# KyleVanMeter/MVOLPS

Hardware: AMD Instinct MI355X
Metric: simplex_pivots_per_s (higher is better)
Workload: dtype f64

## Files before the change

### mvolps_amd/csrc/kernels.hip

```cpp
#include <hip/hip_runtime.h>

#include <cmath>
#include <cstdlib>

#include "kernel_common.hpp"

namespace mvx {

template <int MODE>
__device__ __forceinline__ bool cand_better(const Cand &a, const Cand &b) {
  if (a.idx == 0) return false;
  if (b.idx == 0) return true;
  if (MODE == 0) {
    if (a.k1 > b.k1) return true;
    if (a.k1 < b.k1) return false;
    return a.idx < b.idx;
  } else {
    if (a.k1 < b.k1) return true;
    if (a.k1 > b.k1) return false;
    if (a.k2 > b.k2) return true;
    if (a.k2 < b.k2) return false;
    return a.idx < b.idx;
  }
}
// ... 2389 lines not shown
          if ((spc >> sx) & 1u) {                                                                                        \
            const double ips = s_ip[sx], pvs = s_piv[sx];                                                                \
            _Pragma("unroll") for (int u = 0; u < RPT; u++) a[u] = (ii[u] == lp8[k]) ? ips : xdiv(hc8[u][k], pvs);       \
          } else {                                                                                                       \
            _Pragma("unroll") for (int u = 0; u < RPT; u++) a[u] = (ii[u] == lp8[k]) ? -sq8[k] : fma(-hc8[u][k], sq8[k], a[u]); \
          }                                                                                                              \
        }                                                                                                                \
      }                                                                                                                  \
    }                                                                                                                    \
    s0 += N;                                                                                                             \
  }
      while (gu - s0 >= 8) { COL_BLOCK(8) }
      COL_BLOCK(4)
      COL_BLOCK(2)
      COL_BLOCK(1)
#undef COL_BLOCK
    }
    CH_STAMP(1);
    Cand rb{0.0, 0.0, 0, 0};
    double rp[4] = {a[0], be[0], lb[0], ub[0]}, ro[4];
#pragma unroll
    for (int u = 0; u < RPT; u++) {
      Cand x{0.0, 0.0, 0, 0};
      if (ii[u] <= m) {
        A.colq0[(size_t)g * A.cstride + ii[u]] = a[u];
        if (ratio_row(a[u], sdir, be[u], lb[u], ub[u], 0, A.tol_piv, ii[u], x) && cand_better<1>(x, rb)) {
          rb = x;
          rp[0] = a[u]; rp[1] = be[u]; rp[2] = lb[u]; rp[3] = ub[u];
        }
      }
      HC(g, u) = a[u];
    }
    CH_STAMP(2);
    const Cand pw = xchg<1, 4>(X, rb, rp, ro, s_slots, s_pay);
    if (X.dead) break;
    CH_STAMP(3);
    const int p = pw.idx, p_up = pw.aux;
    const double tstep = pw.k1, piv = ro[0], bp = ro[1], plb = ro[2], pub = ro[3];
    double val[CPT];
#pragma unroll
    for (int u = 0; u < CPT; u++) val[u] = T[(size_t)p * ld + ((jj[u] <= n) ? jj[u] : n)];
    double rcp_l = 0.0;
    if (lane < g) rcp_l = ld_sc1(A.colq0 + (size_t)lane * A.cstride + p);
    bool flip = false;
    double tf = 0.0;
    if (lbq > -INFINITY && ubq < INFINITY && fq != MVX_NF) {
      tf = ubq - lbq;
      if (p == 0 || tf <= tstep) flip = true;
    }
    if (!flip && p == 0) {
      if (lead && g == 0) {
        c->fstate = F_STOP;
        c->phase = PH_PRIMAL2;
      }
      break;
    }
    int kind, lf, stall_new;
    double delta = 0.0, bound = 0.0, s0 = 0.0, xq = 0.0, ip = 1.0;
    if (flip) {
      kind = ST_FLIP;
      lf = (sdir > 0) ? MVX_NU : MVX_NL;
      delta = (sdir > 0) ? tf : -tf;
      stall_new = 0;
#pragma unroll
      for (int u = 0; u < RPT; u++) be[u] = fma(a[u], delta, be[u]);
      z = fma(dq, delta, z);
#pragma unroll
      for (int u = 0; u < CPT; u++) {
        if (jj[u] == q) f[u] = lf;
        sqn[u] = 0.0;
      }
    } else {
      kind = ST_PIVOT;
      bound = p_up ? pub : plb;
      lf = dev_leave_flag(plb, pub, p_up);
      s0 = xdiv(bp - bound, piv);
      xq = dev_nb_value(fq, lbq, ubq);
      ip = xdiv(1.0, piv);
      stall_new = (tstep <= DEGEN_TOL) ? stall + 1 : 0;
#pragma unroll
      for (int u = 0; u < RPT; u++) {
        if (ii[u] == p) {
          be[u] = xq - s0;
          lb[u] = lbq;
          ub[u] = ubq;
        } else
          be[u] = fma(-a[u], s0, be[u]);
      }
      CH_STAMP(4);
      if (lane < g) {
        const double rcp = rcp_l;
        s_wv[wave][0][lane] = rcp;
        s_wv[wave][1][lane] = xdiv(rcp, s_piv[lane]);
      }
      const unsigned spr = (unsigned)__ballot(ispc && s_p[lane < KCH ? lane : 0] == p);
      {
        int s0 = 0;
#define ROW_BLOCK(N)                                                                                                     \
  if (gu - s0 >= N) {                                                                                                    \
    const unsigned bm = ((1u << N) - 1u) << s0;                                                                          \
    double hs8[CPT][N], cp8[N], cd8[N];                                                                                  \
    int lq8[N];                                                                                                          \
    _Pragma("unroll") for (int k = 0; k < N; k++) {                                                                      \
      cp8[k] = s_wv[wave][0][s0 + k];                                                                                    \
      cd8[k] = s_wv[wave][1][s0 + k];                                                                                    \
      lq8[k] = s_q[s0 + k];                                                                                              \
      _Pragma("unroll") for (int u = 0; u < CPT; u++) hs8[u][k] = HS(s0 + k, u);                                         \
    }                                                                                                                    \
    if ((pivm & bm) == bm && (spr & bm) == 0u) {                                                                         \
      _Pragma("unroll") for (int k = 0; k < N; k++) {                                                                    \
        _Pragma("unroll") for (int u = 0; u < CPT; u++) val[u] = (jj[u] == lq8[k]) ? cd8[k] : fma(-cp8[k], hs8[u][k], val[u]); \
      }                                                                                                                  \
    } else {                                                                                                             \
      _Pragma("unroll") for (int k = 0; k < N; k++) {                                                                    \
        const int sx = s0 + k;                                                                                           \
        if ((pivm >> sx) & 1u) {                                                                                         \
          if ((spr >> sx) & 1u) {                                                                                        \
            const double ips = s_ip[sx];                                                                                 \
            _Pragma("unroll") for (int u = 0; u < CPT; u++) val[u] = (jj[u] == lq8[k]) ? ips : -hs8[u][k];               \
          } else {                                                                                                       \
            _Pragma("unroll") for (int u = 0; u < CPT; u++) val[u] = (jj[u] == lq8[k]) ? cd8[k] : fma(-cp8[k], hs8[u][k], val[u]); \
          }                                                                                                              \
        }                                                                                                                \
      }                                                                                                                  \
    }                                                                                                                    \
    s0 += N;                                                                                                             \
  }
        while (gu - s0 >= 8) { ROW_BLOCK(8) }
        ROW_BLOCK(4)
        ROW_BLOCK(2)
        ROW_BLOCK(1)
#undef ROW_BLOCK
      }
      CH_STAMP(5);
#pragma unroll
      for (int u = 0; u < CPT; u++) {
        const int j = jj[u];
        const double sj = xdiv(val[u], piv);
        if (j == q) {
          d[u] = xdiv(dq, piv);
          const double cc = xdiv(wq, piv * piv);
          wgt[u] = cc > 1.0 ? cc : 1.0;
          lbj[u] = plb;
          ubj[u] = pub;
          f[u] = lf;
        } else {
          d[u] = fma(-dq, sj, d[u]);
          const double cc = sj * sj * wq;
          wgt[u] = cc > wgt[u] ? cc : wgt[u];
        }
        if (j <= n) A.srow0[(size_t)g * A.sstride + j] = sj;
        HS(g, u) = sj;
        sqn[u] = sj;
      }
      z = fma(-dq, s0, z);
      if (lead) A.srow0[(size_t)g * A.sstride] = s0;
    }
    s_kind[g] = kind;
    s_p[g] = flip ? 0 : p;
    s_q[g] = q;
    s_piv[g] = flip ? 1.0 : piv;
    s_ip[g] = ip;
    used += flip ? 0 : 1;
    if (lead) {
      c->ch_kind[g] = kind;
      c->ch_p[g] = flip ? 0 : p;
      c->ch_q[g] = q;
      c->ch_lf[g] = lf;
      c->ch_piv[g] = flip ? 1.0 : piv;
      c->ch_xq[g] = xq;
      c->ch_s0[g] = s0;
      c->ch_delta[g] = delta;
      c->ch_elb[g] = lbq;
      c->ch_eub[g] = ubq;
      c->ch_llb[g] = plb;
      c->ch_lub[g] = pub;
      c->ch_bound[g] = bound;
      c->ch_pup[g] = p_up;
      c->ch_stall[g] = stall_new;
      c->ch_cnt[g] = used;
      c->ch_ok[g] = epoch;
    }
    CH_STAMP(6);
    PRICE();
    CH_STAMP(7);
    stall = stall_new;
    g++;
    qc = xchg<0, 5>(X, pc, pp, po, s_slots, s_pay);
    if (dbg && lead) dbg[(size_t)(g - 1) * 16 + 8] = __builtin_amdgcn_s_memrealtime();
  }
#undef PRICE
#undef CH_STAMP
#undef HS
#undef HC
  if (X.dead) {
    if (lead) {
      c->pc_n = 0;
      c->cl_abort = 1;
    }
    return;
  }
  if (g == 0 && fresh) {
#pragma unroll
    for (int u = 0; u < CPT; u++) {
      if (jj[u] <= n) {
        A.pw[0][jj[u]] = 1.0;
        A.pw[1][jj[u]] = 1.0;
      }
    }
  }
  if (g > 0) {
    const int xf = g & 1;
#pragma unroll
    for (int u = 0; u < CPT; u++) {
      if (jj[u] <= n) {
        A.drowk[xf][jj[u]] = d[u];
        A.pwk[xf][jj[u]] = wgt[u];
      }
    }
    if (lead) {
      A.drowk[xf][0] = z;
      A.pwk[xf][0] = 1.0;
    }
  }
  if (lead) {
    c->pc_n = g;
    if (g > 0) {
      c->phase = PH_PRIMAL2;
      c->pc_itlim = end_itlim ? 1 : 0;
    }
  }
}

__device__ void chain_commit(const ChainArgs &A, Ctl *c, int nch) {
  __shared__ int s_cp[KCH], s_cq[KCH], s_ck[KCH], s_rf[KCH], s_cf[KCH], s_R[KCH], s_C[KCH];
  const int t = TIDX;
  const bool on = (t < nch);
  int kind = 0, p = 0, q = 0;
  if (on) {
    kind = c->ch_kind[t];
    p = c->ch_p[t];
    q = c->ch_q[t];
    s_ck[t] = kind;
    s_cp[t] = p;
    s_cq[t] = q;
    s_R[t] = (kind == ST_PIVOT) ? c->bvar[p] : 0;
    s_C[t] = (kind == ST_PIVOT) ? c->nvar[q] : 0;
  }
  __syncthreads();
  bool lastrow = true, lastcol = true, lastflag = true;
  if (on) {
    int rf = t, cf = t;
    for (int u = t - 1; u >= 0; u--) {
      if (s_ck[u] != ST_PIVOT) continue;
      if (s_cp[u] == p) rf = u;
      if (s_cq[u] == q) cf = u;
    }
    s_rf[t] = rf;
    s_cf[t] = cf;
    for (int u = t + 1; u < nch; u++) {
      if (s_cq[u] == q) lastflag = false;
      if (s_ck[u] != ST_PIVOT) continue;
      if (s_cp[u] == p) lastrow = false;
      if (s_cq[u] == q) lastcol = false;
    }
  }
  __syncthreads();
  if (t == 0) {
    for (int u = 0; u < nch; u++) {
      if (s_ck[u] != ST_PIVOT) continue;
      const int a = s_rf[u], b = s_cf[u];
      const int kv = s_R[a];
      s_R[a] = s_C[b];
      s_C[b] = kv;
    }
  }
  __syncthreads();
  if (on) {
    if (kind == ST_PIVOT) {
      if (lastrow) {
        c->bvar[p] = s_R[s_rf[t]];
        A.blb[p] = c->ch_elb[t];
        A.bub[p] = c->ch_eub[t];
      }
      if (lastcol) {
        c->nvar[q] = s_C[s_cf[t]];
        A.nlb[q] = c->ch_llb[t];
        A.nub[q] = c->ch_lub[t];
      }
    }
    if (lastflag) A.nflag[q] = c->ch_lf[t];
  }
  if (t == 0) {
    const int piv_n = c->ch_cnt[nch - 1];
    c->it_cnt += piv_n;
    c->n_flips += nch - piv_n;
    c->n_bulk++;
    if (c->budget > 0) c->budget -= piv_n;
    c->stall = c->ch_stall[nch - 1];
    c->pc_epoch++;
  }
}

typedef const double __attribute__((address_space(4))) *kconst_f64;
template <int TR, int NT>
__global__ __launch_bounds__(256) void k_fbc3(const ChainArgs A) {
  __shared__ double s_cq[KCH][TR];
  Ctl *const c = A.c;
  if (c->done != D_RUN || c->fstate != F_RUN) return;
  const int nch = c->pc_n;
  if (nch == 0) return;
  const int n = A.n;
  const size_t ld = (size_t)A.ld;
  const int j0 = 2 * ((int)blockIdx.x * 256 + TIDX);
  const int i0 = 1 + (int)blockIdx.y * TR;
  const int xf = nch & 1;
  const bool act = (j0 <= n);
  const int jc = act ? j0 : 0;
  double *base = A.T + (size_t)i0 * ld + jc;
  double2 v[TR];
#pragma unroll
  for (int r = 0; r < TR; r++) v[r] = ld2<NT>(reinterpret_cast<const double2 *>(base + (size_t)r * ld));
  unsigned flips = 0;
  for (int l = 0; l < nch; l++) flips |= (c->ch_kind[l] == ST_FLIP) ? (1u << l) : 0u;
  for (int e = TIDX; e < nch * TR; e += 256) {
    const int l = e / TR, r = e % TR;
    s_cq[l][r] = ((flips >> l) & 1u) ? 0.0 : A.colq0[(size_t)l * A.cstride + i0 + r];
  }
  __syncthreads();
  const double *sp = A.srow0 + jc;
  const double *zp = A.zeros + jc;
  for (int l0 = 0; l0 < nch; l0 += 4) {
    double2 s4[4];
#pragma unroll
    for (int k = 0; k < 4; k++) {
      const int lk = (l0 + k < nch) ? l0 + k : nch - 1;
      s4[k] = *reinterpret_cast<const double2 *>(((flips >> lk) & 1u) ? zp : sp + (size_t)lk * A.sstride);
    }
#pragma unroll
    for (int k = 0; k < 4; k++) {
      if (l0 + k < nch) {
#pragma unroll
        for (int r = 0; r < TR; r++) {
          const double ci = s_cq[l0 + k][r];
          asm("v_fma_f64 %0, -%1, %2, %0" : "+v"(v[r].x) : "v"(ci), "v"(s4[k].x));
          asm("v_fma_f64 %0, -%1, %2, %0" : "+v"(v[r].y) : "v"(ci), "v"(s4[k].y));
        }
      }
    }
  }
  if (act) {
    if (j0 == 0) {
#pragma unroll
      for (int r = 0; r < TR; r++) base[(size_t)r * ld + 1] = v[r].y;
    } else {
#pragma unroll
      for (int r = 0; r < TR; r++) st2<NT>(reinterpret_cast<double2 *>(base + (size_t)r * ld), v[r]);
    }
    if (blockIdx.y == 0) {
      *reinterpret_cast<double2 *>(A.T + j0) = *reinterpret_cast<const double2 *>(A.drowk[xf] + j0);
      const double2 w = *reinterpret_cast<const double2 *>(A.pwk[xf] + j0);
      *reinterpret_cast<double2 *>(A.pw[0] + j0) = w;
      *reinterpret_cast<double2 *>(A.pw[1] + j0) = w;
    }
  }
  if (blockIdx.x == 0 && blockIdx.y == 0) chain_commit(A, c, nch);
}

__global__ __launch_bounds__(256) void k_fpatch(const ChainArgs A, int kmax) {
  __shared__ int s_kind[KCH], s_p[KCH], s_q[KCH];
  __shared__ double s_piv[KCH], s_ip[KCH], s_xq[KCH], s_delta[KCH], s_u[KCH];
  Ctl *const c = A.c;
  if (c->done != D_RUN || c->fstate != F_RUN) return;
  const int nch = c->pc_n;
  if (nch == 0) return;
  const int m = A.m, n = A.n;
  const size_t ld = (size_t)A.ld;
  const int job = (int)blockIdx.y, x = (int)blockIdx.x * 256 + TIDX;
  const int jk = (job < kmax) ? 0 : (job < 2 * kmax) ? 1 : 2;
  const int l = (jk == 0) ? job : (jk == 1) ? job - kmax : -1;
  bool live = (jk == 2) || (l < nch && c->ch_kind[l < nch ? l : 0] == ST_PIVOT);
  const int span = (jk == 0) ? n : (jk == 1) ? m : A.mcap1 - 1;
  if ((int)blockIdx.x * 256 > span) live = false;
  if (live) {
    const int lp = (l >= 0) ? c->ch_p[l] : 0, lq = (l >= 0) ? c->ch_q[l] : 0;
    if (TIDX < KCH) {
      const int t = (TIDX < nch) ? TIDX : nch - 1;
      const int kind = c->ch_kind[t];
      const double piv = c->ch_piv[t];
      s_kind[TIDX] = kind;
      s_p[TIDX] = c->ch_p[t];
      s_q[TIDX] = c->ch_q[t];
      s_piv[TIDX] = piv;
      s_ip[TIDX] = (kind == ST_PIVOT) ? xdiv(1.0, piv) : 0.0;
      s_xq[TIDX] = c->ch_xq[t];
      s_delta[TIDX] = c->ch_delta[t];
      s_u[TIDX] = (jk == 0) ? A.colq0[(size_t)t * A.cstride + lp] : A.srow0[(size_t)t * A.sstride + (jk == 1 ? lq : 0)];
    }
    const int xc = (x >= 1 && x <= span) ? x : 1;
    double op[KCH];
#pragma unroll
    for (int t = 0; t < KCH; t++) {
      const int tc = (t < nch) ? t : nch - 1;
      op[t] = (jk == 0) ? A.srow0[(size_t)tc * A.sstride + xc] : A.colq0[(size_t)tc * A.cstride + xc];
    }
    double *dst = (jk == 0) ? A.T + (size_t)lp * ld + xc : A.T + (size_t)xc * ld + (jk == 1 ? lq : 0);
    double val = (jk == 2) ? *dst : 0.0;
    __syncthreads();
    const int i = (jk == 0) ? lp : xc, j = (jk == 0) ? xc : (jk == 1) ? lq : 0;
    const int l0 = (jk == 2) ? 0 : l;
#pragma unroll
    for (int t = 0; t < KCH; t++) {
      if (t >= l0 && t < nch) {
        const double ci = (jk == 0) ? s_u[t] : op[t], sj = (jk == 0) ? op[t] : s_u[t];
        if (s_kind[t] == ST_FLIP) {
          if (j == 0) val = fma(ci, s_delta[t], val);
        } else if (i == s_p[t]) {
          val = (j == s_q[t]) ? s_ip[t] : (j == 0) ? s_xq[t] - sj : -sj;
        } else if (j == s_q[t]) {
          val = xdiv(ci, s_piv[t]);
        } else {
          val = fma(-ci, sj, val);
        }
      }
    }
    if (x >= 1 && x <= span) {
      if (jk != 2 || x <= m) *dst = val;
      if (jk == 2) A.betab[x] = val;
    }
  }
}

__device__ __forceinline__ bool row_violation(double beta, double lb, double ub, double tol, double &viol, int &up) {
  viol = 0.0;
  up = 0;
  if (lb > -INFINITY && beta < lb - tol * (1.0 + fabs(lb))) viol = lb - beta;
  if (ub < INFINITY && beta > ub + tol * (1.0 + fabs(ub))) {
    viol = beta - ub;
    up = 1;
  }
  return viol > 0.0;
}

__device__ __forceinline__ bool dual_ratio_col(double a, double d, int f, int to_upper, double tp, int j, Cand &x) {
  if (f == MVX_NS) return false;
  const double aa = to_upper ? -a : a;
  double r;
  if (aa > tp && (f == MVX_NL || f == MVX_NF)) r = (f == MVX_NF) ? fabs(d) : (d < 0.0 ? -d : 0.0);
  else if (aa < -tp && (f == MVX_NU || f == MVX_NF)) r = (f == MVX_NF) ? fabs(d) : (d > 0.0 ? d : 0.0);
  else return false;
  const double mag = fabs(a);
  x = Cand{xdiv(r, mag), mag, j, 0};
  return true;
}

__global__ __launch_bounds__(DA_THREADS) void k_dboot(Ctl *c) {
  __shared__ Cand lds[17];
  const bool lead = (blockIdx.x == 0 && TIDX == 0);
  if (c->done != D_RUN || c->phase != PH_DUAL || c->stall >= c->stall_limit || c->perturbed) {
    if (lead) c->fstate = F_OFF;
    return;
  }
  const int a = c->curA & 1, m = c->m, n = c->n;
  const size_t ld = (size_t)c->ld;
  const double *T = c->T, *w = c->dwx[a];
  const double tol = c->tol_bnd;
  Cand rb{0.0, 0.0, 0, 0};
  for (int i = 1 + TIDX; i <= m; i += DA_THREADS) {
    double viol;
    int up;
    if (row_violation(T[(size_t)i * ld], c->blb[i], c->bub[i], tol, viol, up)) {
      Cand x{xdiv(viol * viol, w[i]), 0.0, i, up};
      if (cand_better<0>(x, rb)) rb = x;
    }
  }
  rb = block_best<0>(rb, lds);
  const int p2 = rb.idx, p2_up = rb.aux;
  const int j = (int)blockIdx.x * DA_THREADS + TIDX;
  Cand best{0.0, 0.0, 0, 0};
  if (p2 && j >= 1 && j <= n) {
    Cand x{0.0, 0.0, 0, 0};
    if (dual_ratio_col(T[(size_t)p2 * ld + j], c->sgn * T[j], c->nflag[j], p2_up, c->tol_piv, j, x)) best = x;
  }
  __syncthreads();
  best = block_best<1>(best, lds);
  if (TIDX == 0) c->pp[a][blockIdx.x] = best;
  if (lead) {
    c->p_nextx[a] = p2;
    c->p_up_nextx[a] = p2_up;
    c->fstate = F_RUN_DUAL;
    c->step = ST_NONE;
    c->curB = a ^ 1;
    c->npbd = (int)gridDim.x;
  }
}

__global__ __launch_bounds__(DA_THREADS) void k_da(Ctl *c) {
  __shared__ Cand lds[17];
  const int done = c->done, fstate = c->fstate, cur = c->curA, budget = c->budget;
  const int stall = c->stall, stall_limit = c->stall_limit;
  const int npb = c->npbd, m = c->m, n = c->n;
  const size_t ld = (size_t)c->ld;
  double *const T = c->T;
  double *const srow = c->srow;
  const int *const nflag = c->nflag;
  const double *const colq = c->colqx[cur];
  const double *const betac = c->betac[cur];
  const Cand *const pp = c->pp[cur];
  Cand *const ppn = c->pp[cur ^ 1];
  const double *const dwc = c->dwx[cur & 1];
  double *const dwn = c->dwx[(cur & 1) ^ 1];
  const double sgn = c->sgn, tol_bnd = c->tol_bnd, tol_piv = c->tol_piv;
  const int p = c->p_nextx[cur & 1], p_up = c->p_up_nextx[cur & 1];
  if (done != D_RUN || fstate != F_RUN_DUAL) return;
  const bool lead = (blockIdx.x == 0 && TIDX == 0);
  const int lane = TIDX & 63;
  const int j = (int)blockIdx.x * DA_THREADS + TIDX;
  const bool act = (j <= n);
  Cand pc = (lane < npb) ? pp[lane] : Cand{0.0, 0.0, 0, 0};
  const double dold = act ? T[j] : 0.0;
  const int fj = (act && j >= 1) ? nflag[j] : MVX_NS;
  for (int k = lane + 64; k < npb; k += 64) {
    Cand x = pp[k];
    if (cand_better<1>(x, pc)) pc = x;
  }
  pc = wave_bcast_best<1>(pc);
  if (p == 0 || pc.idx == 0 || budget == 0 || stall >= stall_limit) {
    if (lead) c->fstate = F_STOP;
    return;
  }
  const int q = pc.idx;
  const double piv = colq[p], dq = colq[0], wp = dwc[p];
  const double plb = c->blb[p], pub = c->bub[p];
  const double lbq = c->nlb[q], ubq = c->nub[q];
  const int fq = nflag[q];
  const double v = act ? T[(size_t)p * ld + j] : 0.0;
  const double bound = p_up ? pub : plb;
  const int lf = dev_leave_flag(plb, pub, p_up);
  const double xq = dev_nb_value(fq, lbq, ubq);
  const double s0 = xdiv(betac[p] - bound, piv);
  double sj = 0.0, dnew = 0.0;
  if (act) {
    sj = (j == 0) ? s0 : xdiv(v, piv);
    srow[j] = sj;
    dnew = (j == q) ? xdiv(dq, piv) : fma(-dq, sj, dold);
    T[j] = dnew;
  }
  Cand rb{0.0, 0.0, 0, 0};
  for (int i = 1 + TIDX; i <= m; i += DA_THREADS) {
    const double ci = colq[i];
    double beta, lb, ub, w;
    if (i == p) {
      beta = xq - s0;
      lb = lbq;
      ub = ubq;
      const double cc = xdiv(wp, piv * piv);
      w = cc > 1.0 ? cc : 1.0;
    } else {
      beta = fma(-ci, s0, betac[i]);
      lb = c->blb[i];
      ub = c->bub[i];
      const double r = xdiv(ci, piv);
      const double cc = r * r * wp;
      w = dwc[i];
      if (cc > w) w = cc;
    }
    if (blockIdx.x == 0) dwn[i] = w;
    double viol;
    int up;
    if (row_violation(beta, lb, ub, tol_bnd, viol, up)) {
      Cand x{xdiv(viol * viol, w), 0.0, i, up};
      if (cand_better<0>(x, rb)) rb = x;
    }
  }
  rb = block_best<0>(rb, lds);
  const int p2 = rb.idx, p2_up = rb.aux;
  Cand best{0.0, 0.0, 0, 0};
  if (p2 && act && j >= 1) {
    double a2;
    if (p2 == p) a2 = (j == q) ? xdiv(1.0, piv) : -sj;
    else a2 = (j == q) ? xdiv(colq[p2], piv) : fma(-colq[p2], sj, T[(size_t)p2 * ld + j]);
    Cand x{0.0, 0.0, 0, 0};
    if (dual_ratio_col(a2, sgn * dnew, (j == q) ? lf : fj, p2_up, tol_piv, j, x)) best = x;
  }
  __syncthreads();
  best = block_best<1>(best, lds);
  if (TIDX == 0) ppn[blockIdx.x] = best;
  if (lead) {
    c->step = ST_PIVOT;
    c->p = p;
    c->q = q;
    c->p_up = p_up;
    c->piv = piv;
    c->bound = bound;
    c->xq = xq;
    c->leave_flag = lf;
    c->ent_lb = lbq;
    c->ent_ub = ubq;
    c->curB = cur;
    c->stall_new = (pc.k1 <= DEGEN_TOL) ? stall + 1 : 0;
    c->p_nextx[(cur & 1) ^ 1] = p2;
    c->p_up_nextx[(cur & 1) ^ 1] = p2_up;
  }
}

struct PersistArgs {
  Ctl *ctl;
  unsigned long long *head;
  unsigned long long *slot;
  int *abort_flag;
  unsigned long long *dbg;
  int cpw, nw, slot_stride, max_steps;
  int head_stride;
};
constexpr int PMSG_HDR = 16;
constexpr int PERSIST_SPIN = 1 << 20;
constexpr int PERSIST_MAX_CPW = 16;

__device__ __forceinline__ unsigned long long ld_agent(const unsigned long long *p) {
  return __hip_atomic_load(p, __ATOMIC_RELAXED, __HIP_MEMORY_SCOPE_AGENT);
}
__device__ __forceinline__ void st_agent(unsigned long long *p, unsigned long long v) {
  __hip_atomic_store(p, v, __ATOMIC_RELAXED, __HIP_MEMORY_SCOPE_AGENT);
}
__device__ __forceinline__ unsigned long long d2u(double x) { return (unsigned long long)__double_as_longlong(x); }
__device__ __forceinline__ double u2d(unsigned long long x) { return __longlong_as_double((long long)x); }
__device__ __forceinline__ void put_word(unsigned long long *g, unsigned long long v, unsigned tag) {
  const unsigned long long t = (unsigned long long)tag << 32;
  st_agent(g, t | (v >> 32));
  st_agent(g + 1, t | (v & 0xffffffffull));
}
__device__ __forceinline__ bool persist_aborted(const int *abort_flag) {
  return __hip_atomic_load(abort_flag, __ATOMIC_RELAXED, __HIP_MEMORY_SCOPE_AGENT) != 0;
}

template <int NW>
__device__ __forceinline__ bool get_words(const unsigned long long *g, int first, int stride, int count, unsigned tag, const int *abort_flag,
                                          unsigned long long (&out)[NW]) {
  unsigned pending = 0;
#pragma unroll
  for (int k = 0; k < NW; k++)
    if (first + k * stride < count) pending |= 1u << k;
  for (int spin = 0; pending && spin < PERSIST_SPIN; spin++) {
    unsigned long long a[NW], b[NW];
#pragma unroll
    for (int k = 0; k < NW; k++)
      if (pending & (1u << k)) {
        const unsigned long long *p = g + 2 * (size_t)(first + k * stride);
        a[k] = ld_agent(p);
        b[k] = ld_agent(p + 1);
      }
#pragma unroll
// ... 116 lines not shown
        }
        for (int i = TIDX; i < R; i += 256) st_agent(myslot + PMSG_HDR + i, d2u(col[i]));
        asm volatile("s_waitcnt vmcnt(0)" ::: "memory");
      }
      __syncthreads();
      if (TIDX == 0) {
        unsigned long long *g = a.head + ((size_t)(tag & 1) * a.nw + w) * a.head_stride;
        put_word(g, d2u(best.k1), tag);
        put_word(g + 2, ((unsigned long long)(unsigned)best.idx << 1) | (best.aux > 0 ? 1ull : 0ull), tag);
      }
    }
    const long long c1 = clock64();
    t_prop += c1 - c0;
    if (TIDX < 64) {
      const unsigned long long *g = a.head + (size_t)(tag & 1) * a.nw * a.head_stride;
      unsigned pend = 0;
#pragma unroll
      for (int k = 0; k < 16; k++)
        if (TIDX + 64 * (k >> 2) < a.nw) pend |= 1u << k;
      bool good = true;
      for (int spin = 0; spin < PERSIST_SPIN; spin++) {
        unsigned long long v[16];
        n_sweeps++;
#pragma unroll
        for (int k = 0; k < 16; k++)
          if (pend & (1u << k)) v[k] = ld_agent(g + (size_t)(TIDX + 64 * (k >> 2)) * a.head_stride + (k & 3));
#pragma unroll
        for (int k = 0; k < 16; k++)
          if ((pend & (1u << k)) && (unsigned)(v[k] >> 32) == tag) {
            s_gran[4 * (TIDX + 64 * (k >> 2)) + (k & 3)] = (unsigned)v[k];
            pend &= ~(1u << k);
          }
        if (spin == 0) t_first += clock64() - c1;
        if (__all(pend == 0)) break;
        if ((spin & 63) == 63) {
          if (persist_aborted(a.abort_flag)) {
            good = false;
            break;
          }
          __builtin_amdgcn_s_sleep(1);
        }
        if (spin == PERSIST_SPIN - 1) good = false;
      }
      const int allgood = __all(good ? 1 : 0);
      Cand best{0.0, 0.0, 0, 0};
      if (allgood) {
        for (int st = TIDX; st < a.nw; st += 64) {
          const unsigned long long sc = ((unsigned long long)s_gran[4 * st] << 32) | s_gran[4 * st + 1];
          const unsigned long long mt = ((unsigned long long)s_gran[4 * st + 2] << 32) | s_gran[4 * st + 3];
          const int idx = (int)(mt >> 1);
          if (idx) {
            Cand x{u2d(sc), 0.0, idx, (mt & 1ull) ? 1 : -1};
            if (cand_better<0>(x, best)) best = x;
          }
        }
      }
      best = wave_best<0>(best);
      if (TIDX == 0) {
        lds[16] = best;
        s_ok = allgood;
      }
    }
    __syncthreads();
    if (!s_ok) {
      ok = false;
      break;
    }
    const long long c2 = clock64();
    t_gath += c2 - c1;
    const Cand ent = lds[16];
    const int q = ent.idx;
    if (q == 0 || budget == 0 || stall >= stall_limit || steps >= a.max_steps) break;
    const int owner = (q - 1) / cpw;
    {
      const unsigned long long *ws = a.slot + ((size_t)(tag & 1) * a.nw + owner) * a.slot_stride;
      if (TIDX >= 1 && TIDX <= 12) s_hdr[TIDX] = ld_agent(ws + TIDX);
      if (owner == w) {
        const double *col = tile + (size_t)(q - j0) * R;
        for (int i = TIDX; i < R; i += 256) colq[i] = col[i];
      } else {
        for (int i0 = 0; i0 < R; i0 += 1024) {
          unsigned long long v[4];
#pragma unroll
          for (int k = 0; k < 4; k++)
            if (i0 + TIDX + 256 * k < R) v[k] = ld_agent(ws + PMSG_HDR + i0 + TIDX + 256 * k);
#pragma unroll
          for (int k = 0; k < 4; k++)
            if (i0 + TIDX + 256 * k < R) colq[i0 + TIDX + 256 * k] = u2d(v[k]);
        }
      }
      __syncthreads();
    }
    const long long c3 = clock64();
    t_read += c3 - c2;
    const int kind = (int)s_hdr[1];
    if (kind == ST_STOP) break;
    const int p = (int)(unsigned)(s_hdr[2] & 0xffffffffull);
    const double piv = u2d(s_hdr[3]), bound = u2d(s_hdr[4]), xq = u2d(s_hdr[5]), ent_lb = u2d(s_hdr[6]), ent_ub = u2d(s_hdr[7]);
    const double delta = u2d(s_hdr[8]), wq = u2d(s_hdr[9]), step_len = u2d(s_hdr[11]);
    const int ent_var = (int)(unsigned)s_hdr[10], newflag = (int)(unsigned)s_hdr[12];
    if (kind == ST_FLIP) {
      for (int i = TIDX; i < R; i += 256) beta[i] = fma(colq[i], delta, beta[i]);
      if (owner == w && TIDX == q - j0) my_nflag = newflag;
      n_flips++;
      stall = 0;
      it++;
      __syncthreads();
      continue;
    }
    const double s0 = xdiv(beta[p] - bound, piv);
    if (TIDX < nc) {
      const int j = j0 + TIDX;
      double *col = tile + (size_t)TIDX * R;
      const double s_own = xdiv(col[p], piv);
      s_sc[TIDX] = s_own;
      const double dq = colq[0];
      col[0] = (j == q) ? xdiv(dq, piv) : fma(-dq, s_own, col[0]);
      if (j == q) {
        const double cc = xdiv(wq, piv * piv);
        my_w = cc > 1.0 ? cc : 1.0;
      } else {
        const double cc = s_own * s_own * wq;
        my_w = cc > my_w ? cc : my_w;
      }
    }
    const int lv_var = bvar[p];
    const double lv_lb = blb[p], lv_ub = bub[p];
    if (owner == w && TIDX == q - j0) {
      my_nvar = lv_var;
      my_nlb = lv_lb;
      my_nub = lv_ub;
      my_nflag = newflag;
    }
    __syncthreads();
    double sc[PERSIST_MAX_CPW];
    for (int cc = 0; cc < nc; cc++) sc[cc] = s_sc[cc];
    const int cq = (owner == w) ? q - j0 : -1;
    for (int i = 1 + TIDX; i < R; i += 256) {
      const double ci = colq[i];
      if (i == p) {
        for (int cc = 0; cc < nc; cc++) tile[(size_t)cc * R + i] = -sc[cc];
        beta[i] = xq - s0;
      } else {
        for (int cc = 0; cc < nc; cc++) {
          double *e = tile + (size_t)cc * R + i;
          *e = fma(-ci, sc[cc], *e);
        }
        beta[i] = fma(-ci, s0, beta[i]);
      }
      if (cq >= 0) tile[(size_t)cq * R + i] = (i == p) ? xdiv(1.0, piv) : xdiv(ci, piv);
    }
    if (TIDX == 0) {
      beta[0] = fma(-colq[0], s0, beta[0]);
      bvar[p] = ent_var;
      blb[p] = ent_lb;
      bub[p] = ent_ub;
    }
    it_cnt++;
    if (budget > 0) budget--;
    stall = (step_len <= DEGEN_TOL) ? stall + 1 : 0;
    steps++;
    it++;
    __syncthreads();
    t_appl += clock64() - c3;
  }
  if (TIDX == 0 && a.dbg && steps > 0) {
    const unsigned long long work = (unsigned long long)((t_prop + t_read + t_appl) / steps), gat = (unsigned long long)(t_gath / steps);
    atomicMax(&a.dbg[8], work);
    atomicMax(&a.dbg[9], ~work);
    atomicMax(&a.dbg[10], gat);
    atomicMax(&a.dbg[11], ~gat);
  }
  if (w == 0 && TIDX == 0 && a.dbg) {
    a.dbg[0] += (unsigned long long)t_prop; a.dbg[1] += (unsigned long long)t_gath; a.dbg[2] += (unsigned long long)t_read;
    a.dbg[3] += (unsigned long long)t_appl; a.dbg[4] += (unsigned long long)steps;
    a.dbg[5] += (unsigned long long)n_sweeps; a.dbg[6] += (unsigned long long)t_first;
  }
  if (!ok && TIDX == 0) __hip_atomic_store(a.abort_flag, 1, __ATOMIC_RELAXED, __HIP_MEMORY_SCOPE_AGENT);
  __syncthreads();
  for (int i = TIDX; i < R; i += 256) {
    double *row = c->T + (size_t)i * ld;
    for (int cc = 0; cc < nc; cc++) row[j0 + cc] = tile[(size_t)cc * R + i];
    if (w == 0) {
      row[0] = beta[i];
      if (i) {
        c->bvar[i] = bvar[i];
        c->blb[i] = blb[i];
        c->bub[i] = bub[i];
      }
    }
  }
  if (TIDX < nc) {
    c->nvar[j0 + TIDX] = my_nvar;
    c->nflag[j0 + TIDX] = my_nflag;
    c->nlb[j0 + TIDX] = my_nlb;
    c->nub[j0 + TIDX] = my_nub;
    pw_g[j0 + TIDX] = my_w;
  }
  if (w == 0 && TIDX == 0) {
    c->it_cnt = it_cnt;
    c->n_flips = n_flips;
    c->stall = stall;
    c->budget = budget;
    c->step = ST_NONE;
  }
}

size_t persist_lds_bytes(int m, int cpw) { return ((size_t)(m + 1) * (size_t)(cpw + 4)) * 8 + (size_t)(m + 1) * 4 + 64; }
int persist_max_cpw() { return PERSIST_MAX_CPW; }
int persist_slot_words(int m_cap) { return (PMSG_HDR + m_cap + 1 + 31) / 32 * 32; }
int launch_persist(Ctl *d_ctl, unsigned long long *head, unsigned long long *slot, int *abort_flag, unsigned long long *dbg, int m, int cpw, int nw,
                   int slot_stride, int max_steps, int head_stride, hipStream_t s) {
  static size_t attr_bytes = 0;
  const size_t lds = persist_lds_bytes(m, cpw);
  if (lds > attr_bytes) {
    if (hipFuncSetAttribute(reinterpret_cast<const void *>(k_persist), hipFuncAttributeMaxDynamicSharedMemorySize, (int)lds) != hipSuccess) {
      (void)hipGetLastError();
      return -1;
    }
    attr_bytes = lds;
  }
  PersistArgs a;
  a.ctl = d_ctl; a.head = head; a.slot = slot; a.abort_flag = abort_flag; a.dbg = dbg;
  a.cpw = cpw; a.nw = nw; a.slot_stride = slot_stride; a.max_steps = max_steps;
  a.head_stride = head_stride;
  hipLaunchKernelGGL(k_persist, dim3((unsigned)nw), dim3(256), lds, s, a);
  return hipGetLastError() == hipSuccess ? 0 : -1;
}


static int g_tr = 0, g_hot = 1, g_nt = -1;
void set_tuning(int tr, int hot, int nt) {
  g_tr = (tr == 4 || tr == 8 || tr == 16 || tr == 32) ? tr : 0;
  g_hot = hot ? 1 : 0;
  g_nt = (nt >= 0 && nt <= 2) ? nt : -1;
}
static int pick_nt(int m, int n) {
  if (g_nt >= 0) return g_nt;
  const size_t bytes = (size_t)(m + 1) * (size_t)((n + 1 + LD_ALIGN - 1) / LD_ALIGN * LD_ALIGN) * 8;
  if (bytes > NT_THRESHOLD_BYTES) return 1;
  return (bytes >= WT_MIN_BYTES && bytes <= WT_MAX_BYTES) ? 2 : 0;
}
static int pick_tr(int m, int n) {
  if (g_tr) return g_tr;
  const long tiles = ((n + 2) / 2 + 255) / 256;
  if ((long)((m + 15) / 16) * tiles >= 2048) return 16;
  if ((long)((m + 7) / 8) * tiles >= 2048) return 8;
  return 4;
}
int fused_npb(int n) { return (n + 1 + 255) / 256; }
int fused_nrb_max(int m) { return (m + 3) / 4; }
int chain_ncb(int n) { return fused_npb(n); }
int chain_nrb(int m) { return (m + 255) / 256; }
void launch_pboot(const ChainArgs &a, hipStream_t s) {
  hipLaunchKernelGGL(k_pboot, dim3(a.ncb > a.nrb ? a.ncb : a.nrb), dim3(256), 0, s, a);
}
void launch_pstep(const ChainArgs &a, int g, hipStream_t s) {
  hipLaunchKernelGGL(k_pc, dim3(a.nrb), dim3(256), 0, s, a, g);
  hipLaunchKernelGGL(k_pr, dim3(a.ncb), dim3(256), 0, s, a, g);
}
void launch_pc(const ChainArgs &a, int g, hipStream_t s) { hipLaunchKernelGGL(k_pc, dim3(a.nrb), dim3(256), 0, s, a, g); }
int chain_cluster_nw(int m, int n) {
  const int span = m > n ? m : n;
  int nw = (span + 255) / 256;
  if (nw > 32) nw = 32;
  return nw < 1 ? 1 : nw;
}
int chain_cluster_kmax(int m, int n) {
  const int nw = chain_cluster_nw(m, n), tt = nw * 256;
  const int cpt = (n + tt - 1) / tt, rpt = (m + tt - 1) / tt;
  if (cpt > 2 || rpt > 2) return 0;
  const int per_step = (cpt > 1 || rpt > 1 ? 4 : 2) * 256 * 8;
  const int k = (140 * 1024) / per_step;
  return k > KCH ? KCH : k;
}
int launch_chain(const ChainArgs &a, hipStream_t s) {
  const int tt = a.nw * 256;
  const int cpt = (a.n + tt - 1) / tt, rpt = (a.m + tt - 1) / tt;
  const bool wide = (cpt > 1 || rpt > 1);
  const size_t lds = (size_t)(a.kmax > 0 ? a.kmax : 1) * (wide ? 4 : 2) * 256 * 8;
  static size_t attr1 = 0, attr2 = 0;
  size_t &attr = wide ? attr2 : attr1;
  const void *fn = wide ? reinterpret_cast<const void *>(k_chain<2, 2>) : reinterpret_cast<const void *>(k_chain<1, 1>);
  if (lds > attr) {
    if (hipFuncSetAttribute(fn, hipFuncAttributeMaxDynamicSharedMemorySize, (int)lds) != hipSuccess) {
      (void)hipGetLastError();
      return -1;
    }
    attr = lds;
  }
  if (wide) hipLaunchKernelGGL((k_chain<2, 2>), dim3(8 * a.nw), dim3(256), lds, s, a);
  else hipLaunchKernelGGL((k_chain<1, 1>), dim3(8 * a.nw), dim3(256), lds, s, a);
  return 0;
}
void launch_fpatch(const ChainArgs &a, int steps, hipStream_t s) {
  const int span = a.mcap1 > a.n + 1 ? a.mcap1 : a.n + 1;
  hipLaunchKernelGGL(k_fpatch, dim3((span + 255) / 256, 2 * steps + 1), dim3(256), 0, s, a, steps);
}
void launch_fbc3(const ChainArgs &a, int steps, hipStream_t s) {
  const int m = a.m, n = a.n;
  const int pairs = (n + 2) / 2;
  int tr = pick_tr(m, n);
  if (tr > 16) tr = 16;
  if (!g_tr && tr == 16 && steps >= 12) tr = 8;
  const int nt = pick_nt(m, n);
  dim3 grid((pairs + 255) / 256, (m + tr - 1) / tr);
#define FBC2_CASE(TR_, NT_) \
  if (tr == TR_ && nt == NT_) { hipLaunchKernelGGL((k_fbc3<TR_, NT_>), grid, dim3(256), 0, s, a); return; }
  FBC2_CASE(16, 0) FBC2_CASE(16, 1) FBC2_CASE(16, 2) FBC2_CASE(8, 0) FBC2_CASE(8, 1) FBC2_CASE(8, 2) FBC2_CASE(4, 0) FBC2_CASE(4, 1) FBC2_CASE(4, 2)
#undef FBC2_CASE
  std::abort();
}
void launch_dboot(Ctl *d_ctl, int n, hipStream_t s) { hipLaunchKernelGGL(k_dboot, dim3((n + DA_THREADS) / DA_THREADS), dim3(DA_THREADS), 0, s, d_ctl); }
void launch_da(Ctl *d_ctl, int n, hipStream_t s) { hipLaunchKernelGGL(k_da, dim3((n + DA_THREADS) / DA_THREADS), dim3(DA_THREADS), 0, s, d_ctl); }
void launch_db(Ctl *d_ctl, int m, int n, hipStream_t s) {
  const int pairs = (n + 2) / 2;
  const int tr = pick_tr(m, n);
  const int nt = pick_nt(m, n);
  dim3 grid((pairs + 255) / 256, (m + tr - 1) / tr);
#define DB_CASE(TR_, NT_) \
  if (tr == TR_ && nt == NT_) { hipLaunchKernelGGL((k_fb<TR_, 1, NT_, 1>), grid, dim3(256), 0, s, d_ctl); return; }
  DB_CASE(16, 0) DB_CASE(16, 1) DB_CASE(8, 0) DB_CASE(8, 1) DB_CASE(4, 0) DB_CASE(4, 1) DB_CASE(32, 0) DB_CASE(32, 1)
  DB_CASE(16, 2) DB_CASE(8, 2) DB_CASE(4, 2) DB_CASE(32, 2)
#undef DB_CASE
  std::abort();
}
int launch_dsel(Ctl *d_ctl, int m, int n, hipStream_t s, int slots) {
  static int state = -1;
  if (state < 0) {
    const char *e = std::getenv("MVX_DSEL");
    if (e && e[0] == '0') state = 0;
    else if (hipFuncSetAttribute(reinterpret_cast<const void *>(k_dsel), hipFuncAttributeMaxDynamicSharedMemorySize, (int)DSEL_LDS) == hipSuccess) state = 1;
    else {
      (void)hipGetLastError();
      state = 0;
    }
  }
  if (state != 1 || m > 1024 || n > 1024) return 0;
  hipLaunchKernelGGL(k_dsel, dim3(1, 1, slots), dim3(1024), DSEL_LDS, s, d_ctl);
  return 1;
}
void launch_select(Ctl *d_ctl, hipStream_t s, int slots) {
  BatchQueue q{};
  hipLaunchKernelGGL(k_select, dim3(1, 1, slots), dim3(1024), 0, s, d_ctl, q);
}
void launch_select_queue(Ctl *d_ctl, const BatchQueue &q, hipStream_t s, int slots) {
  hipLaunchKernelGGL(k_select, dim3(1, 1, slots), dim3(1024), 0, s, d_ctl, q);
}
void launch_update(Ctl *d_ctl, int m, int n, hipStream_t s, int slots, int chained, int busy_slots) {
  const int pairs = (n + 2) / 2;
  const long tiles = (pairs + 255) / 256;
  const long work = busy_slots > 0 ? std::min(busy_slots, slots) : slots;
  int tr = ((long)((m + 16) / 16) * tiles * work >= 2048) ? 16 : ((long)((m + 8) / 8) * tiles * work >= 2048) ? 8 : 4;
  static const int tr_cap = std::getenv("MVX_UPD_TR") ? std::atoi(std::getenv("MVX_UPD_TR")) : 4;
  if (slots > 1 && chained && tr > tr_cap) tr = tr_cap >= 16 ? 16 : tr_cap >= 8 ? 8 : 4;
  dim3 grid((unsigned)tiles, (m + tr) / tr, slots);
  const int nt = (tr == 16) ? pick_nt(m, n) : 0;
  if (nt == 1) hipLaunchKernelGGL((k_update<16, 1>), grid, dim3(256), 0, s, d_ctl, chained);
  else if (nt == 2) hipLaunchKernelGGL((k_update<16, 2>), grid, dim3(256), 0, s, d_ctl, chained);
  else if (tr == 16) hipLaunchKernelGGL((k_update<16, 0>), grid, dim3(256), 0, s, d_ctl, chained);
  else if (tr == 8) hipLaunchKernelGGL((k_update<8, 0>), grid, dim3(256), 0, s, d_ctl, chained);
  else hipLaunchKernelGGL((k_update<4, 0>), grid, dim3(256), 0, s, d_ctl, chained);
}
void launch_p1_head(Ctl *d_ctl, hipStream_t s) { hipLaunchKernelGGL(k_p1_head, dim3(1), dim3(1024), 0, s, d_ctl); }
void launch_p1_select(Ctl *d_ctl, hipStream_t s) { hipLaunchKernelGGL(k_p1_select, dim3(1), dim3(1024), 0, s, d_ctl); }
__global__ __launch_bounds__(64) void k_scatter_ctl(Ctl *dst, const Ctl *src, const int *idx, int count) {
  const int t = (int)blockIdx.x;
  if (t >= count) return;
  const unsigned *s = reinterpret_cast<const unsigned *>(&src[t]);
  unsigned *d = reinterpret_cast<unsigned *>(&dst[idx[t]]);
  for (int w = TIDX; w < (int)(sizeof(Ctl) / 4); w += 64) d[w] = s[w];
}
void launch_scatter_ctl(Ctl *dst, const Ctl *src, const int *idx, int count, hipStream_t s) {
  hipLaunchKernelGGL(k_scatter_ctl, dim3(count), dim3(64), 0, s, dst, src, idx, count);
}
__global__ __launch_bounds__(256) void k_copy_many(CopyBatch b) {
  const CopyJob j = b.jobs[blockIdx.y];
  const uint4 *__restrict__ src = reinterpret_cast<const uint4 *>(j.src);
  uint4 *__restrict__ dst = reinterpret_cast<uint4 *>(j.dst);
  const size_t n = j.bytes >> 4;
  constexpr int U = 8;
  for (size_t base = (size_t)blockIdx.x * (256 * U); base < n; base += (size_t)gridDim.x * (256 * U)) {
    uint4 v[U];
#pragma unroll
    for (int u = 0; u < U; u++) {
      const size_t i = base + (size_t)u * 256 + TIDX;
      if (i < n) v[u] = src[i];
    }
#pragma unroll
    for (int u = 0; u < U; u++) {
      const size_t i = base + (size_t)u * 256 + TIDX;
      if (i < n) dst[i] = v[u];
    }
  }
}
void launch_copy_many(const CopyBatch &b, hipStream_t s) {
  size_t mx = 0;
  for (int k = 0; k < b.count; k++) mx = b.jobs[k].bytes > mx ? b.jobs[k].bytes : mx;
  const size_t per_block = (size_t)256 * 8 * 16;
  unsigned gx = (unsigned)((mx + per_block - 1) / per_block);
  if (gx > 1024) gx = 1024;
  if (gx < 1) gx = 1;
  hipLaunchKernelGGL(k_copy_many, dim3(gx, (unsigned)b.count), dim3(256), 0, s, b);
}
void launch_p1_fix(Ctl *d_ctl, int n, hipStream_t s) { hipLaunchKernelGGL(k_p1_fix, dim3((n + 1 + 255) / 256), dim3(256), 0, s, d_ctl); }
void launch_rowcomb(Ctl *d_ctl, int m, int n, int respect_done, hipStream_t s) {
  const int nchunks = (m + ROWCOMB_CHUNK - 1) / ROWCOMB_CHUNK;
  dim3 grid((n + 1 + 255) / 256, nchunks > 0 ? nchunks : 1);
  hipLaunchKernelGGL(k_rowcomb_partial, grid, dim3(256), 0, s, d_ctl, respect_done);
  hipLaunchKernelGGL(k_rowcomb_final, dim3((n + 1 + 255) / 256), dim3(256), 0, s, d_ctl, respect_done, nchunks);
}
void launch_shift_nonbasic(double *T, int ld, int m, int jj, double delta, hipStream_t s) {
  hipLaunchKernelGGL(k_shift_nonbasic, dim3((m + 1 + 255) / 256), dim3(256), 0, s, T, ld, m, jj, delta);
}
void launch_set_basic_bounds(double *blb, double *bub, int i, double lb, double ub, hipStream_t s) {
  hipLaunchKernelGGL(k_set_basic_bounds, dim3(1), dim3(64), 0, s, blb, bub, i, lb, ub);
}
void launch_set_nonbasic(double *nlb, double *nub, int *nflag, int j, double lb, double ub, int flag, hipStream_t s) {
  hipLaunchKernelGGL(k_set_nonbasic, dim3(1), dim3(64), 0, s, nlb, nub, nflag, j, lb, ub, flag);
}
void launch_add_rows(double *T, int ld, int n, int *bvar, double *blb, double *bub, int *nvar, int first, int nrs, int m_new,
                     hipStream_t s) {
  int span = (n > m_new ? n : m_new) + 1;
  hipLaunchKernelGGL(k_add_rows, dim3((span + 255) / 256), dim3(256), 0, s, T, ld, n, bvar, blb, bub, nvar, first, nrs);
}
void launch_export(Ctl *d_ctl, unsigned char *stage, int m, int n, int force, hipStream_t s, int slots, size_t slot_stride) {
  int span = (n > m ? n : m) + 1;
  hipLaunchKernelGGL(k_export, dim3((span + 255) / 256, 1, slots), dim3(256), 0, s, d_ctl, stage, force, slot_stride);
}

}
```

Measured before the change: 57890.

## Software-pipeline pivot-row fetches and prefetch column coefficients in bulk-chain update

Restructures the k_fbc3 rank-update kernel. Column coefficients are loaded into registers before the tile load, and flip flags are built with a wavefront ballot instead of a serial loop. The pivot-row loads are double-buffered in groups of two with branchless zero-row selection and sched barriers, so global loads overlap the FMAs. The launcher also stops dropping the tile height to 8 for long chains. The price is more registers and fixed-size unrolled prefetch rounds, and the ballot assumes the chain length fits in one 64-lane wavefront.

```diff
diff --git a/mvolps_amd/csrc/kernels.hip b/mvolps_amd/csrc/kernels.hip
--- a/mvolps_amd/csrc/kernels.hip
+++ b/mvolps_amd/csrc/kernels.hip
@@ -2715,10 +2715,14 @@
   }
 }
 
-typedef const double __attribute__((address_space(4))) *kconst_f64;
+typedef double f64x2 __attribute__((ext_vector_type(2)));
+typedef const f64x2 __attribute__((address_space(1))) *gconst_f64x2;
 template <int TR, int NT>
 __global__ __launch_bounds__(256) void k_fbc3(const ChainArgs A) {
-  __shared__ double s_cq[KCH][TR];
+  constexpr int G = 2;
+  constexpr int ROUNDS = (KCH * TR + 255) / 256;
+  constexpr int SROWS = (ROUNDS * 256 / TR > KCH) ? ROUNDS * 256 / TR : KCH;
+  __shared__ double s_cq[SROWS][TR];
   Ctl *const c = A.c;
   if (c->done != D_RUN || c->fstate != F_RUN) return;
   const int nch = c->pc_n;
@@ -2731,36 +2735,65 @@
   const bool act = (j0 <= n);
   const int jc = act ? j0 : 0;
   double *base = A.T + (size_t)i0 * ld + jc;
+  const int lane = TIDX & 63;
+  const int kind = c->ch_kind[lane < nch ? lane : nch - 1];
+  double cq[ROUNDS];
+#pragma unroll
+  for (int k = 0; k < ROUNDS; k++) {
+    const int l = (TIDX + 256 * k) / TR, r = TIDX % TR;
+    cq[k] = A.colq0[(size_t)(l < nch ? l : nch - 1) * A.cstride + i0 + r];
+  }
+  __builtin_amdgcn_sched_barrier(0);
   double2 v[TR];
 #pragma unroll
   for (int r = 0; r < TR; r++) v[r] = ld2<NT>(reinterpret_cast<const double2 *>(base + (size_t)r * ld));
-  unsigned flips = 0;
-  for (int l = 0; l < nch; l++) flips |= (c->ch_kind[l] == ST_FLIP) ? (1u << l) : 0u;
-  for (int e = TIDX; e < nch * TR; e += 256) {
-    const int l = e / TR, r = e % TR;
-    s_cq[l][r] = ((flips >> l) & 1u) ? 0.0 : A.colq0[(size_t)l * A.cstride + i0 + r];
-  }
-  __syncthreads();
-  const double *sp = A.srow0 + jc;
-  const double *zp = A.zeros + jc;
-  for (int l0 = 0; l0 < nch; l0 += 4) {
-    double2 s4[4];
-#pragma unroll
-    for (int k = 0; k < 4; k++) {
-      const int lk = (l0 + k < nch) ? l0 + k : nch - 1;
-      s4[k] = *reinterpret_cast<const double2 *>(((flips >> lk) & 1u) ? zp : sp + (size_t)lk * A.sstride);
-    }
-#pragma unroll
-    for (int k = 0; k < 4; k++) {
+  __builtin_amdgcn_sched_barrier(0);
+  const unsigned flips = (unsigned)__ballot(kind == ST_FLIP);
+#pragma unroll
+  for (int k = 0; k < ROUNDS; k++) {
+    const int l = (TIDX + 256 * k) / TR, r = TIDX % TR;
+    s_cq[l][r] = ((flips >> (l < nch ? l : nch - 1)) & 1u) ? 0.0 : cq[k];
+  }
+  const uintptr_t sp = reinterpret_cast<uintptr_t>(A.srow0), zp = reinterpret_cast<uintptr_t>(A.zeros);
+  auto fetch = [&](double2(&s)[G], int l0) {
+#pragma unroll
+    for (int k = 0; k < G; k++) {
+      const bool in = (l0 + k < nch);
+      const int lk = (l0 + k) & (KCH - 1);
+      const uintptr_t fl = (uintptr_t)0 - (uintptr_t)(in ? ((flips >> lk) & 1u) : 1u);
+      const uintptr_t row = (zp & fl) | ((sp + (uintptr_t)lk * A.sstride * sizeof(double)) & ~fl);
+      const f64x2 t = *((gconst_f64x2)row + (in ? jc / 2 : 0));
+      s[k] = make_double2(t.x, t.y);
+    }
+  };
+  auto apply = [&](const double2(&s)[G], int l0) {
+#pragma unroll
+    for (int k = 0; k < G; k++) {
       if (l0 + k < nch) {
 #pragma unroll
         for (int r = 0; r < TR; r++) {
           const double ci = s_cq[l0 + k][r];
-          asm("v_fma_f64 %0, -%1, %2, %0" : "+v"(v[r].x) : "v"(ci), "v"(s4[k].x));
-          asm("v_fma_f64 %0, -%1, %2, %0" : "+v"(v[r].y) : "v"(ci), "v"(s4[k].y));
+          asm("v_fma_f64 %0, -%1, %2, %0" : "+v"(v[r].x) : "v"(ci), "v"(s[k].x));
+          asm("v_fma_f64 %0, -%1, %2, %0" : "+v"(v[r].y) : "v"(ci), "v"(s[k].y));
         }
       }
     }
+  };
+  double2 sa[G], sb[G];
+  fetch(sa, 0);
+  __builtin_amdgcn_sched_barrier(0);
+  fetch(sb, G);
+  __builtin_amdgcn_sched_barrier(0);
+  __syncthreads();
+  for (int l0 = 0; l0 < nch; l0 += 2 * G) {
+    apply(sa, l0);
+    __builtin_amdgcn_sched_barrier(0);
+    fetch(sa, l0 + 2 * G);
+    __builtin_amdgcn_sched_barrier(0);
+    apply(sb, l0 + G);
+    __builtin_amdgcn_sched_barrier(0);
+    fetch(sb, l0 + 3 * G);
+    __builtin_amdgcn_sched_barrier(0);
   }
   if (act) {
     if (j0 == 0) {
@@ -3483,7 +3516,7 @@
   const int pairs = (n + 2) / 2;
   int tr = pick_tr(m, n);
   if (tr > 16) tr = 16;
-  if (!g_tr && tr == 16 && steps >= 12) tr = 8;
+  (void)steps;
   const int nt = pick_nt(m, n);
   dim3 grid((pairs + 255) / 256, (m + tr - 1) / tr);
 #define FBC2_CASE(TR_, NT_) \
```

Measured after the change: 56930. 1.6% lower.
